# oxfordcontrol/Clarabel.jl

Hardware: AMD Instinct MI355X
Metric: IPM iterations/sec + KKT factor+solve ms, 10k-var sparse QP, 1/2/4/8 GPU (higher is better)
Workload: dtype f64; 1 GPU; random sparse QP n=10000 m=20000 NN cone, uniform pattern (cfg 2a); N=30000, nnzK=99990, nnzL=16225495, supernodes=20125, levels=97, ordering=minimum degree, parallelism=1 independent problem(s), one per GPU

## Files before the change

clarabel.jl_amd/csrc/dense_tile.h:

```cpp
#pragma once
#include <hip/hip_runtime.h>
#include <stdint.h>

#include "device_plan.h"
#include "kernel_util.h"

namespace hipkkt {

template <int NT, int NR>
struct DenseRaw {
    double a[NT], b[NR], d;
};

template <int NT, int NR>
__device__ __forceinline__ void dense_load(DenseRaw<NT, NR> &f, const double *sp, const double *dv, const unsigned (&coff)[NT],
                                           const unsigned (&roff)[NR], unsigned r8, int K, int k0, int lk) {
    int kk = k0 + lk;
    kk = kk < K ? kk : K - 1;
    const unsigned ko = (unsigned)kk * r8;
#ifdef HIPKKT_EXPERIMENT_NOLOAD
    f.d = 1.0 + ko * 1e-9;
#pragma unroll
    for (int t = 0; t < NT; t++) f.a[t] = 1e-3 * (coff[t] + 1);
#pragma unroll
    for (int t = 0; t < NR; t++) f.b[t] = 1e-3 * (roff[t] + 1);
#else
    f.d = ld_off(dv, (unsigned)kk * 8u);
#pragma unroll
    for (int t = 0; t < NT; t++) f.a[t] = ld_off(sp, coff[t] + ko);
#pragma unroll
    for (int t = 0; t < NR; t++) f.b[t] = ld_off(sp, roff[t] + ko);
#endif
}

template <int NT, int NR>
__device__ __forceinline__ void dense_mma(const DenseRaw<NT, NR> &f, v4f64 (&acc)[NT][NR], unsigned mbits, int K, int k0, int lk) {
    const double dk = (k0 + lk < K) ? -f.d : 0.0;
    double a[NT], b[NR];
#pragma unroll
    for (int t = 0; t < NT; t++)
        a[t] = ((mbits >> t) & 1u) ? f.a[t] * dk : 0.0;
#pragma unroll
    for (int t = 0; t < NR; t++) b[t] = ((mbits >> (4 + t)) & 1u) ? f.b[t] : 0.0;
#pragma unroll
    for (int tj = 0; tj < NT; tj++)
#pragma unroll
        for (int ti = 0; ti < NR; ti++)
            acc[tj][ti] = __builtin_amdgcn_mfma_f64_16x16x4f64(a[tj], b[ti], acc[tj][ti], 0, 0, 0);
}

template <int NT, int NR, bool DEEP = false>
__device__ __forceinline__ void dense_tile_core(const DevPlan &P, double *tp, int rt, int nrt, int wt, int task_begin,
                                                int task_end, int lane, int tj0, int ti0) {
    const int l15 = lane & 15, lk = lane >> 4;

    v4f64 acc[NT][NR];
#pragma unroll
    for (int tj = 0; tj < NT; tj++)
#pragma unroll
        for (int reg = 0; reg < 4; reg++) {
            const int jj = (tj0 + tj) * 16 + lk + 4 * reg;
#pragma unroll
            for (int ti = 0; ti < NR; ti++) {
                const int ii = (ti0 + ti) * 16 + l15;
                const bool ok = ii < nrt && jj < wt;
                const double v = ld_off(tp, ok ? (unsigned)(ii + jj * rt) * 8u : 0u);
                acc[tj][ti][reg] = ok ? v : 0.0;
            }
        }

    const int last = task_end - 1;
    auto gm_of = [&](int q, int &g_, int &m_) { const DenseTask *t = P.dtasks + (q < last ? q : last); g_ = t->geom; m_ = t->map; };
    auto req_maps = [&](int geom_u, int map_u, int (&mr_)[NR], int (&mc_)[NT]) {
        const int16_t *tm = P.upd_tmap + (int64_t)((geom_u & (1 << 17)) ? map_u : 0) * 128;
#pragma unroll
        for (int x = 0; x < NR; x++) mr_[x] = tm[(ti0 + x) * 16 + l15];
#pragma unroll
        for (int x = 0; x < NT; x++) mc_[x] = tm[64 + (tj0 + x) * 16 + l15];
    };
    DenseTask Tc = P.dtasks[task_begin];
    int mr[NR], mc[NT], g1, m1;
    req_maps(rfl(Tc.geom), rfl(Tc.map), mr, mc);
    gm_of(task_begin + 1, g1, m1);
    for (int q = task_begin; q < task_end; q++) {
        const DenseTask Tn = P.dtasks[q + 1 < task_end ? q + 1 : q];
        int g2, m2, mrn[NR], mcn[NT];
        gm_of(q + 2, g2, m2);
        req_maps(rfl(g1), rfl(m1), mrn, mcn);
        const int row_lo = rfl(Tc.row_lo), nrows = rfl(Tc.nrows), col_lo = rfl(Tc.col_lo), ncols = rfl(Tc.ncols),
                  geom = rfl(Tc.geom), K = rfl(Tc.K);
        const unsigned r8 = (unsigned)rfl(Tc.r8);
        const double *sp = rfl_ptr(P.Lx + Tc.panel_off);
        const double *dv = rfl_ptr(P.D + Tc.dfirst);
        const int c_r = geom & 255, c_c = (geom >> 8) & 255;
        unsigned roff[NR], coff[NT], mbits = 0;
        if (geom & (1 << 17)) {
#pragma unroll
            for (int x = 0; x < NR; x++) {
                const int m = mr[x];
                roff[x] = (unsigned)(row_lo + (m >= 0 ? m : 0)) * 8u;
                mbits |= m >= 0 ? 16u << x : 0u;
            }
#pragma unroll
            for (int x = 0; x < NT; x++) {
                const int m = mc[x];
                coff[x] = (unsigned)(col_lo + (m >= 0 ? m : 0)) * 8u;
                mbits |= m >= 0 ? 1u << x : 0u;
            }
        } else {
#pragma unroll
            for (int x = 0; x < NR; x++) {
                const int ii = (ti0 + x) * 16 + l15 - c_r;
                const bool okr = ii >= 0 && ii < nrows;
                roff[x] = (unsigned)(row_lo + (okr ? ii : 0)) * 8u;
                mbits |= okr ? 16u << x : 0u;
            }
#pragma unroll
            for (int x = 0; x < NT; x++) {
                const int jj = (tj0 + x) * 16 + l15 - c_c;
                const bool okc = jj >= 0 && jj < ncols;
                coff[x] = (unsigned)(col_lo + (okc ? jj : 0)) * 8u;
                mbits |= okc ? 1u << x : 0u;
            }
        }
        if (NT == 1 || DEEP) {
            DenseRaw<NT, NR> f0, f1, f2, f3;
            dense_load<NT, NR>(f0, sp, dv, coff, roff, r8, K, 0, lk);
            dense_load<NT, NR>(f1, sp, dv, coff, roff, r8, K, 4, lk);
            dense_load<NT, NR>(f2, sp, dv, coff, roff, r8, K, 8, lk);
            dense_load<NT, NR>(f3, sp, dv, coff, roff, r8, K, 12, lk);
            for (int k0 = 0; k0 < K; k0 += 16) {
                __builtin_amdgcn_sched_barrier(0);
                dense_mma<NT, NR>(f0, acc, mbits, K, k0, lk);
                dense_load<NT, NR>(f0, sp, dv, coff, roff, r8, K, k0 + 16, lk);
                __builtin_amdgcn_sched_barrier(0);
                dense_mma<NT, NR>(f1, acc, mbits, K, k0 + 4, lk);
                dense_load<NT, NR>(f1, sp, dv, coff, roff, r8, K, k0 + 20, lk);
                __builtin_amdgcn_sched_barrier(0);
                dense_mma<NT, NR>(f2, acc, mbits, K, k0 + 8, lk);
                dense_load<NT, NR>(f2, sp, dv, coff, roff, r8, K, k0 + 24, lk);
                __builtin_amdgcn_sched_barrier(0);
                dense_mma<NT, NR>(f3, acc, mbits, K, k0 + 12, lk);
                dense_load<NT, NR>(f3, sp, dv, coff, roff, r8, K, k0 + 28, lk);
            }
        } else {
            DenseRaw<NT, NR> fa, fb;
            dense_load<NT, NR>(fa, sp, dv, coff, roff, r8, K, 0, lk);
            for (int k0 = 0; k0 < K; k0 += 8) {
                dense_load<NT, NR>(fb, sp, dv, coff, roff, r8, K, k0 + 4, lk);
                __builtin_amdgcn_sched_barrier(0);
                dense_mma<NT, NR>(fa, acc, mbits, K, k0, lk);
                __builtin_amdgcn_sched_barrier(0);
                dense_load<NT, NR>(fa, sp, dv, coff, roff, r8, K, k0 + 8, lk);
                __builtin_amdgcn_sched_barrier(0);
                if (k0 + 4 < K) dense_mma<NT, NR>(fb, acc, mbits, K, k0 + 4, lk);
                __builtin_amdgcn_sched_barrier(0);
            }
        }
        Tc = Tn;
        g1 = g2; m1 = m2;
#pragma unroll
        for (int x = 0; x < NR; x++) mr[x] = mrn[x];
#pragma unroll
        for (int x = 0; x < NT; x++) mc[x] = mcn[x];
    }
#pragma unroll
    for (int tj = 0; tj < NT; tj++)
#pragma unroll
        for (int reg = 0; reg < 4; reg++) {
            const int jj = (tj0 + tj) * 16 + lk + 4 * reg;
#pragma unroll
            for (int ti = 0; ti < NR; ti++) {
                const int ii = (ti0 + ti) * 16 + l15;
                if (ii < nrt && jj < wt) st_off(tp, (unsigned)(ii + jj * rt) * 8u, acc[tj][ti][reg]);
            }
        }
}

__device__ __forceinline__ void dense_tile_core_full(const DevPlan &P, double *tp, int rt, int task_begin, int task_end, int lane) {
    const int l15 = lane & 15, lk = lane >> 4;
    v4f64 acc[4][4];
#pragma unroll
    for (int tj = 0; tj < 4; tj++)
#pragma unroll
        for (int reg = 0; reg < 4; reg++) {
            const int jj = tj * 16 + lk + 4 * reg;
#pragma unroll
// ... 56 lines not shown
                advance();
            } else if (q + 1 < task_end) {
                const DenseTask Tc = Tn;
                Tn = P.dtasks[q + 2 < task_end ? q + 2 : q + 1];
                setup(Tc);
                load(fa);
                advance();
            }
            __builtin_amdgcn_sched_barrier(0);
            mma(fb);
            __builtin_amdgcn_sched_barrier(0);
        }
    }
#pragma unroll
    for (int tj = 0; tj < 4; tj++)
#pragma unroll
        for (int reg = 0; reg < 4; reg++) {
            const int jj = tj * 16 + lk + 4 * reg;
#pragma unroll
            for (int ti = 0; ti < 4; ti++) st_off(tp, (unsigned)(ti * 16 + l15 + jj * rt) * 8u, acc[tj][ti][reg]);
        }
}

template <int NT, int NR, bool DEEP = false>
__device__ __forceinline__ void dense_tile(const DevPlan &P, const DenseGroup *Gp, int lane, int tj0, int ti0) {
    const DenseGroup G = *Gp;
    const int task_begin = rfl(G.task_begin), task_end = rfl(G.task_end);
    const int wt = rfl(G.wt);
    if (tj0 * 16 >= wt) return;
    const int rt = rfl(G.rt);
    double *tp = rfl_ptr(P.Lx + G.tile_off);
    const int nrt = rfl(G.nrt);
    if (ti0 * 16 >= nrt) return;
    if (NT == 4 && NR == 4 && (rfl(G.pad) & 1)) {
        dense_tile_core_full(P, tp, rt, task_begin, task_end, lane);
        return;
    }
    dense_tile_core<NT, NR, DEEP>(P, tp, rt, nrt, wt, task_begin, task_end, lane, tj0, ti0);
}

__device__ __forceinline__ void dense_extra_tiles(const DevPlan &P, int begin, int count, int xb, int per_wave) {
    const int lane = threadIdx.x & 63;
    int idx = rfl((xb * 4 + (int)(threadIdx.x >> 6)) * per_wave);
    for (int q = 0; q < per_wave && idx < count; q++, idx++) dense_tile<4, 4, true>(P, P.dgroups + begin + idx, lane, 0, 0);
}

}
```

clarabel.jl_amd/csrc/hipkkt_abi.cpp:

```cpp
#include "hipkkt_internal.h"

using namespace hipkkt;
using namespace hipkkt_host;

namespace hipkkt_host {
thread_local std::string g_create_error;
DebugOpts &debug_opts() { static DebugOpts o; return o; }
bool verbose() { static const bool v = getenv("HIPKKT_VERBOSE") != nullptr; return v; }
}

extern "C" {

void hipkkt_default_opts(hipkkt_opts *o) {
    if (!o) return;
    memset(o, 0, sizeof(*o));
    o->index_base = 0;
    o->supernode_max_width = kMaxSnWidth;
    o->relax_supernodes = 1;
    o->update_policy = 2;
    o->update_batch = 0;
    o->front_min_panels = 0;
    o->dynamic_reg_eps = 1e-13;
    o->dynamic_reg_delta = 2e-7;
    o->amd_dense_scale = 1.5;
// ... 670 lines not shown
    else if (k == "FB_V2") o.fb_v2 = !is0();
    else if (k == "FORCE_TWIN") o.force_twin = is1();
    else if (k == "NO_GRAPH") o.no_graph = is1();
    else if (k == "NO_PERSIST") o.no_persist = is1();
    else if (k == "FULL_TILES") o.full_tiles = !is0();
    else if (k == "FRONT_BLOCK") o.front_block = !is0();
    else if (k == "SPLIT_K") o.split_k = !is0();
    else if (k == "GATHER_OVERLAP") o.gather_overlap = !is0();
    else if (k == "GATHER_SORT") o.gather_sort = !is0();
    else if (k == "GATHER_SIDE_BLOCKS") { if (!value) o.gather_side_blocks = def.gather_side_blocks; else if (num(&v) && v >= 0) o.gather_side_blocks = (int)v; else return HIPKKT_ERR_ARGUMENT; }
    else if (k == "DENSE_TRI") o.dense_tri = !is0();
    else if (k == "ORDERING") o.ordering_amd = value && value[0] == 'a';
    else if (k == "NO_FRONT") o.no_front = is1();
    else if (k == "HOST_ASSEMBLY") o.host_assembly = is1();
    else if (k == "FRONT_BLOCK_MIN_ROWS") { if (!value) o.front_block_min_rows = def.front_block_min_rows; else if (num(&v)) o.front_block_min_rows = (int)v; else return HIPKKT_ERR_ARGUMENT; }
    else if (k == "SUPERHOP") { if (!value) o.superhop = def.superhop; else if (num(&v)) o.superhop = (int)v; else return HIPKKT_ERR_ARGUMENT; }
    else if (k == "DEBUG_FLAGS") { if (!value) o.debug_flags = 0; else if (num(&v)) o.debug_flags = (int)v; else return HIPKKT_ERR_ARGUMENT; }
    else if (k == "SPIN_LIMIT") { if (!value) o.spin_limit = def.spin_limit; else if (num(&v) && v >= 0) o.spin_limit = (long long)v; else return HIPKKT_ERR_ARGUMENT; }
    else if (k == "PERSIST_RETRY") { if (!value) o.persist_retry = def.persist_retry; else if (num(&v) && v >= 0) o.persist_retry = (long long)v; else return HIPKKT_ERR_ARGUMENT; }
    else if (k == "ACCURATE") {
        if (!value) o.accurate = def.accurate;
        else if (!num(&v)) return HIPKKT_ERR_ARGUMENT;
        else o.accurate = v == 0.0 ? 1e300 : v;
    } else if (k == "PSD_LARGE_MIN") {
        if (!value) o.psd_large_min = def.psd_large_min;
        else if (!num(&v) || v < 0 || v > 128 || v != (double)(int)v) return HIPKKT_ERR_ARGUMENT;
        else o.psd_large_min = v == 0.0 ? def.psd_large_min : (int)v;
    } else if (k == "FB_EXTRA_PW") {
        o.fb_extra_pw = def.fb_extra_pw; o.fb_pen1 = def.fb_pen1; o.fb_pen2 = def.fb_pen2;
        if (value) {
            int m = o.fb_extra_pw; double a = o.fb_pen1, b = o.fb_pen2;
            if (sscanf(value, "%d,%lf,%lf", &m, &a, &b) < 1) return HIPKKT_ERR_ARGUMENT;
            o.fb_extra_pw = std::max(1, std::min(m, 2)); o.fb_pen1 = a; o.fb_pen2 = b;
        }
    } else {
        g_create_error = "hipkkt_debug_set: unknown switch " + k;
        return HIPKKT_ERR_ARGUMENT;
    }
    return HIPKKT_OK;
#endif
}

const char *hipkkt_last_error(hipkkt_handle h) { return h ? h->err.c_str() : g_create_error.c_str(); }

}
```

clarabel.jl_amd/csrc/hipkkt_factor.cpp:

```cpp
#include "hipkkt_internal.h"

using namespace hipkkt;
using namespace hipkkt_host;

namespace hipkkt_host {

static double slot_value(const hipkkt_solver *S, int slot) {
    double v;
    memcpy(&v, (const char *)S->h_scal + slot * sizeof(double), sizeof(double));
    return v;
}

static void read_scalars(hipkkt_solver *S) {
    HK_CHECK(hipMemcpyAsync(S->h_flags, S->dp.flags, FL_COUNT * sizeof(int), hipMemcpyDeviceToHost, S->stream));
    HK_CHECK(hipMemcpyAsync(S->h_scal, S->dp.scal, SC_COUNT * sizeof(double), hipMemcpyDeviceToHost, S->stream));
    HK_CHECK(hipStreamSynchronize(S->stream));
}


static void enqueue_factor_level(hipkkt_solver *S, int l) {
    const HostPlan &P = S->plan;
    const int n = P.fac_lvl_ptr[l + 1] - P.fac_lvl_ptr[l];
    if (P.fac_lvl_maxw[l] <= 8)
        launch_factor_level(S->stream, S->dp, P.fac_lvl_ptr[l], n, P.fac_lvl_maxw[l], S->opts.dynamic_reg_eps,
                            S->opts.dynamic_reg_delta);
    else
        launch_factor_panel(S->stream, S->dp, P.fac_lvl_ptr[l], n, S->opts.dynamic_reg_eps, S->opts.dynamic_reg_delta);
}

static void enqueue_front_batch(hipkkt_solver *S, const FrontBatch &B) {
#ifdef HIPKKT_TESTING
    if (!S->fb.sw.v2) {
        launch_front_block(S->stream, S->dp, B, S->fb.d_sync, S->fb.d_scratch, S->fb.d_stream, S->opts.dynamic_reg_eps,
                           S->opts.dynamic_reg_delta, S->fb.sw.streamed, S->fb.d_trace);
        return;
    }
#endif
    launch_front_block2(S->stream, S->dp, B, S->fb.d_sync, S->fb.d_scratch, S->fb.d_stream, S->opts.dynamic_reg_eps,
                        S->opts.dynamic_reg_delta, S->fb.d_trace);
}

static void enqueue_split_k(hipkkt_solver *S, int l) {
    if (S->split.group_count[l] <= 0) return;
    launch_update_dense(S->stream, S->dp, S->split.group_begin[l], S->split.group_count[l], false);
    launch_split_reduce(S->stream, S->dp, S->split.d_recs + S->split.rec_ptr[l], S->split.rec_ptr[l + 1] - S->split.rec_ptr[l]);
}

static void enqueue_gather(hipkkt_solver *S, int l) {
    const HostPlan &P = S->plan;
    const int64_t e0 = P.gath_stage_ptr[l], n = P.gath_stage_ptr[l + 1] - e0, h0 = S->split.heavy_ptr[l], nh = S->split.heavy_ptr[l + 1] - h0;
    const int64_t head = S->split.gath[l];
    if (head < 0 || S->side_join_level >= 0) { launch_update_gather(S->stream, S->dp, e0, n, h0, nh); return; }
    const int64_t hh = S->split.gath_heavy[l];
    launch_update_gather(S->stream, S->dp, e0, head, h0, hh);
    HK_CHECK(hipEventRecord(S->ev_fork, S->stream));
    HK_CHECK(hipStreamWaitEvent(S->idle_stream, S->ev_fork, 0));
    launch_update_gather(S->idle_stream, S->dp, e0 + head, n - head, h0 + hh, nh - hh, debug_opts().gather_side_blocks);
    HK_CHECK(hipEventRecord(S->ev_join, S->idle_stream));
    S->side_join_level = l + P.update_batch_used;
}
static void join_side(hipkkt_solver *S, int l) {
    if (S->side_join_level < 0 || l < S->side_join_level) return;
    HK_CHECK(hipStreamWaitEvent(S->stream, S->ev_join, 0));
    S->side_join_level = -1;
}

struct Riders { int count = 0, begin = 0, per_wave = 1; };
// ... 52 lines not shown
        T.prof_dense4_ms = 0; T.prof_dense4_flops = 0; T.prof_dense4_launches = (int)dense.size();
        T.prof_launch_ms.clear(); T.prof_launch_flops.clear(); T.prof_launch_tiles.clear();
        for (const DenseLaunch &d : dense) {
            const double t = ms(d.t);
            T.prof_dense4_ms += t;
            T.prof_dense4_flops += d.flops;
            T.prof_launch_ms.push_back(t);
            T.prof_launch_flops.push_back(d.flops);
            T.prof_launch_tiles.push_back(d.tiles);
        }
        T.prof_fb_ms = 0; T.prof_fb_launches = (int)batches.size(); T.prof_fb_panels = fb_panels; T.prof_fb_flops = fb_flops;
        for (const Span &s : batches) T.prof_fb_ms += ms(s);
        T.prof_extra_tiles = extra_tiles; T.prof_extra_flops = extra_flops;
    }
};

static void enqueue_updates(hipkkt_solver *S, int l, const Riders &x, FactorProbe *probe) {
    const HostPlan &P = S->plan;
    hipStream_t st = S->stream;
    const int g0 = P.upd_stage_ptr[l], nd = P.upd_stage_ndense[l], ng = P.upd_stage_ngather[l];
    if (P.upd_stage_ptr[l + 1] == g0) probe = nullptr;
    if (probe) probe->stage_begin(x);
    join_side(S, l);
    launch_update_dense(st, S->dp, g0, nd - x.count, dense_full_k(nd, P.upd_stage_flops_dense[l]));
    enqueue_split_k(S, l);
    if (probe) probe->dense_end(l, nd - x.count);
    enqueue_gather(S, l);
    launch_update_stage(st, S->dp, g0 + nd + ng, P.upd_stage_ptr[l + 1] - g0 - nd - ng);
    if (probe) probe->stage_end();
}

static double dense_stage_cost_us(int m) {
    if (m <= 0) return 0.0;
    if (m <= kDenseStripTiles) return 20.0 + 0.065 * m;
    if (m <= 768) return 66.0;
    const int k = m / 1024, rem = m % 1024;
    const double base = k == 0 ? 0.0 : k == 1 ? 77.0 : 65.0 * k;
    if (rem == 0) return base;
    if (rem <= 256) return base + 13.0;
    if (rem <= 512) return base + 20.0;
    return k == 0 ? 77.0 : 65.0 * (k + 1);
}
static int fb_extra_tiles_of_stage(int nd, int ncrit, int next_blk, int *per_wave_out) {
    constexpr int cus = 254, rmin = 64;
    const DebugOpts &dbo = debug_opts();
    const int pw_max = dbo.fb_extra_pw;
    const double pen[3] = {0.0, dbo.fb_pen1, dbo.fb_pen2};
// ... 193 lines not shown
```

clarabel.jl_amd/csrc/hipkkt_internal.h:

```cpp
#pragma once
#include "../../include/hipkkt.h"

#include <hip/hip_runtime.h>

#include <algorithm>
#include <atomic>
#include <chrono>
#include <cmath>
#include <cstdlib>
#include <cstring>
#include <deque>
#include <functional>
#include <future>
#include <memory>
#include <mutex>
#include <new>
#include <string>
#include <thread>
#include <vector>

#include "assemble.h"
#include "cone_layout.h"
#include "device_plan.h"
#include "hipkkt_cones.h"
// ... 35 lines not shown
    bool fb_stream = true;
    bool fb_v2 = true;
    bool force_twin = false;
    bool no_graph = false;
    bool no_persist = false;
    bool full_tiles = true;
    bool front_block = true;
    bool split_k = true;
    bool gather_overlap = true;
    bool gather_sort = true;
    int gather_side_blocks = 512;
    bool dense_tri = true;
    bool ordering_amd = false;
    bool no_front = false;
    bool host_assembly = false;
    int front_block_min_rows = -1;
    int superhop = -1;
    int debug_flags = 0;
    long long spin_limit = -1;
    long long persist_retry = -1;
    double accurate = 64.0;
    int fb_extra_pw = 1;
    double fb_pen1 = 10.0, fb_pen2 = 28.0;
    int psd_large_min = 65;
};
DebugOpts &debug_opts();
bool verbose();

struct GraphSlot {
    hipGraphExec_t exec = nullptr;
    bool valid = false;
    int static_enable = -1;
    double eps_const = 0, eps_prop = 0;
};

}

using namespace hipkkt;
using namespace hipkkt_host;

struct RefineOpts {
    int32_t enable; double reltol, abstol; int64_t max_iter; double stop_ratio;
    bool same_graph(const RefineOpts &o) const { return reltol == o.reltol && abstol == o.abstol && max_iter == o.max_iter && stop_ratio == o.stop_ratio; }
};

constexpr int kNumCtx = 2;
// ... 24 lines not shown
    bool l1 = false;
    KKTImage img;
    HostPlan plan;
    PlanOptions plan_opts;
    SolveSchedule sched;
    DevPlan dp{};
    std::vector<std::pair<void *, size_t>> allocs;
    std::string err;

    int N = 0;
    int64_t nnzK = 0;
    std::chrono::steady_clock::time_point t_created{};
    PersistState persist;
    FrontBatchState fb;
    UpdateSplit split;
    SocTables soc;
    ResidualBuffers res;
    ReducedSolve red;
    TwinState twin;
    SolverStats stats;
    ConeState cones;
    double accurate_threshold = 64.0;
    int last_npolish = 0;
    int inv_nsmall = 0, inv_wsmall = 1, inv_nwide = 0;
    int side_join_level = -1;
    hipEvent_t ev_fork = nullptr, ev_join = nullptr;

    int64_t *d_mapHs = nullptr, *d_mapP = nullptr, *d_mapA = nullptr, *d_diag_full = nullptr;
    std::vector<int64_t> cone_numel;
    std::vector<int32_t> cone_hs_dense, cone_sparse_kind;

    double *d_stage = nullptr;
    int64_t *d_stage_idx = nullptr;
    int64_t stage_cap = 0;
    double *h_scal = nullptr;
    double *h_scal_red = nullptr;
    int *h_flags = nullptr;

    hipkkt_host::GraphSlot g_factor;
    bool use_graph = true;
    bool runtime_ready = false;
    bool profiling = false;
    bool profiling_no_extra = false;
    hipEvent_t ev0 = nullptr, ev1 = nullptr, ev2 = nullptr, ev3 = nullptr;
    bool kval_event_pending = false;
    double last_eps = 0;
// ... 129 lines not shown
```

clarabel.jl_amd/csrc/hipkkt_setup.cpp:

```cpp
#include "hipkkt_internal.h"

using namespace hipkkt;
using namespace hipkkt_host;

namespace hipkkt_host {

namespace {
struct PlanCache {
    struct Entry {
        uint64_t key;
        std::string optkey;
        std::vector<int64_t> colptr, rowval;
        std::shared_ptr<const HostPlan> plan;
    };
    std::mutex mu;
    std::deque<Entry> entries;
    int64_t hits = 0, misses = 0;
    static constexpr size_t kMaxEntries = 8;
    static constexpr int64_t kMaxNnzL = 40000000;
    static PlanCache &get() { static PlanCache c; return c; }
    static bool enabled() { return debug_opts().plan_cache; }
    static uint64_t fnv(uint64_t h, const void *p, size_t n) {
        const unsigned char *b = (const unsigned char *)p;
        for (size_t i = 0; i < n; i++) { h ^= b[i]; h *= 1099511628211ull; }
// ... 16 lines not shown
};
}
void plan_cache_counts(int64_t *hits, int64_t *misses) {
    PlanCache &c = PlanCache::get();
    std::lock_guard<std::mutex> lk(c.mu);
    *hits = c.hits; *misses = c.misses;
}

void init_runtime(hipkkt_solver *S) {
    HK_CHECK(hipSetDevice(S->device));
    RuntimePool &rp = RuntimePool::get();
    auto need = [&](void *p) { if (!p) throw DeviceError{"creating a stream / event / pinned buffer failed"}; return p; };
    S->stream = (hipStream_t)need(rp.stream_get(S->device, 0));
    S->idle_stream = (hipStream_t)need(rp.stream_get(S->device, 1));
    {
        const DebugOpts &o = debug_opts();
        S->fb.sw.extra = o.fb_extra;
        S->fb.sw.streamed = o.fb_stream;
        S->fb.sw.v2 = o.fb_v2 && S->fb.sw.streamed;
#ifndef HIPKKT_TESTING
        S->fb.sw.streamed = S->fb.sw.v2 = true;
#endif
        S->accurate_threshold = o.accurate;
        S->twin.force = o.force_twin;
    }
    static_assert(SC_COUNT * sizeof(double) <= RuntimePool::kPinned && sizeof(RefineState) <= RuntimePool::kPinned, "pinned chunk too small");
    for (hipEvent_t *e : {&S->ev0, &S->ev1, &S->ev2, &S->ev3, &S->ev_fork, &S->ev_join}) *e = (hipEvent_t)need(rp.event_get(S->device));
    S->h_scal = (double *)need(rp.pinned_alloc(S->device));
    S->h_flags = (int *)need(rp.pinned_alloc(S->device));
    S->h_scal_red = S->h_scal + 16;
    static_assert((16 + kScalRedDoubles) * sizeof(double) <= RuntimePool::kPinned, "pinned chunk too small for the reduced-solve scalars");
    memset(S->h_scal, 0, SC_COUNT * sizeof(double));
    memset(S->h_flags, 0, FL_COUNT * sizeof(int));
    if (debug_opts().no_graph) S->use_graph = false;
    for (int c = 0; c < kNumCtx; c++) {
        SolveCtx &C = S->ctx[c];
        if (c == 0) C.stream = S->stream;
        else { C.stream = (hipStream_t)need(rp.stream_get(S->device, 2)); C.own_stream = true; }
        C.ev_a = (hipEvent_t)need(rp.event_get(S->device));
        C.ev_b = (hipEvent_t)need(rp.event_get(S->device));
        C.h_rs = (RefineState *)need(rp.pinned_alloc(S->device));
        C.h_flags = (int *)need(rp.pinned_alloc(S->device));
        memset(C.h_rs, 0, sizeof(RefineState));
        memset(C.h_flags, 0, FL_COUNT * sizeof(int));
    }
}
// ... 536 lines not shown
```

clarabel.jl_amd/csrc/kernel_util.h:

```cpp
#pragma once
#include <hip/hip_runtime.h>
#include <stdint.h>

namespace hipkkt {

static inline unsigned nblk(int64_t n, int bs = 256) { return (unsigned)((n + bs - 1) / bs); }

typedef double v4f64 __attribute__((ext_vector_type(4)));

__device__ __forceinline__ double readlane_f64(double x, int l) {
    const unsigned long long u = (unsigned long long)__double_as_longlong(x);
    const unsigned lo = __builtin_amdgcn_readlane((unsigned)u, l), hi = __builtin_amdgcn_readlane((unsigned)(u >> 32), l);
    return __longlong_as_double((long long)(((unsigned long long)hi << 32) | lo));
}
__device__ __forceinline__ int rfl(int v) { return __builtin_amdgcn_readfirstlane(v); }

template <class T>
__device__ __forceinline__ T *rfl_ptr(T *p) {
    const unsigned long long u = (unsigned long long)p;
    const unsigned lo = __builtin_amdgcn_readfirstlane((unsigned)u), hi = __builtin_amdgcn_readfirstlane((unsigned)(u >> 32));
    return (T *)(((unsigned long long)hi << 32) | lo);
}
#define HK_GLOBAL __attribute__((address_space(1)))
__device__ __forceinline__ double ld_off(const double *base, unsigned byte_off) {
    return *(const HK_GLOBAL double *)((const HK_GLOBAL char *)base + byte_off);
}
__device__ __forceinline__ void st_off(double *base, unsigned byte_off, double v) {
    *(HK_GLOBAL double *)((HK_GLOBAL char *)base + byte_off) = v;
}

__device__ __forceinline__ int ld_relaxed_i(const int *p) { return __hip_atomic_load(p, __ATOMIC_RELAXED, __HIP_MEMORY_SCOPE_AGENT); }
__device__ __forceinline__ double ld_relaxed(const double *p) { return __hip_atomic_load(p, __ATOMIC_RELAXED, __HIP_MEMORY_SCOPE_AGENT); }
__device__ __forceinline__ void st_relaxed(double *p, double v) { __hip_atomic_store(p, v, __ATOMIC_RELAXED, __HIP_MEMORY_SCOPE_AGENT); }

__device__ __forceinline__ double pivot_rcp(double d) {
    double r = __builtin_amdgcn_rcp(d);
    r = fma(fma(-d, r, 1.0), r, r);
    r = fma(fma(-d, r, 1.0), r, r);
    return r;
}

__device__ __forceinline__ double pivot_rcp3(double d) {
    const double r = __builtin_amdgcn_rcp(d);
    const double e = fma(-d, r, 1.0);
    const double e2 = fma(e, e, e);
    return fma(r, e2, r);
// ... 38 lines not shown
```

clarabel.jl_amd/csrc/kernels.h:

```cpp
#pragma once
#include <hip/hip_runtime.h>

#include "device_plan.h"

namespace hipkkt {
void launch_scatter_values(hipStream_t st, double *kval, const int64_t *idx, const double *vals, int64_t n, double scale);
void launch_scale_values(hipStream_t st, double *kval, const int64_t *idx, int64_t n, double scale);
void launch_soc_batch(hipStream_t st, double *kval, const int64_t *uidx, const int64_t *vidx, const int *cone_of,
                      const double *u, const double *v, const double *eta2, int64_t n, const int64_t *didx, int nsoc);
void launch_psd_hs(hipStream_t st, double *kval, const int64_t *map_hs, int64_t hs_off, const double *W, int n, const int *skip = nullptr);
void launch_zero_words(hipStream_t st, void *p, int nwords);
void launch_maxabs_gather(hipStream_t st, const double *v, const int64_t *idx, int64_t n, unsigned long long *slot);
void launch_init_panels(hipStream_t st, const DevPlan &P, int64_t nnz, int static_enable, double eps_const, double eps_prop);
void launch_factor_level(hipStream_t st, const DevPlan &P, int item_begin, int nitems, int wmax, double dyn_eps, double dyn_delta);
void launch_factor_panel(hipStream_t st, const DevPlan &P, int item_begin, int nitems, double dyn_eps, double dyn_delta);
void launch_update_stage(hipStream_t st, const DevPlan &P, int group_begin, int ngroups);
constexpr int kDenseStripTiles = 384;
constexpr double kFullKFlopsPerTile = 1.5e6;
inline bool dense_full_k(int nd, double flops) { return nd > 0 && flops >= kFullKFlopsPerTile * nd; }
void launch_update_dense(hipStream_t st, const DevPlan &P, int group_begin, int ngroups, bool full_k = false);
void launch_split_reduce(hipStream_t st, const DevPlan &P, const SplitRec *recs, int n);
void launch_update_gather(hipStream_t st, const DevPlan &P, int64_t ebegin, int64_t n, int64_t hbegin, int64_t nheavy, int max_blocks = 0);
void launch_invert_diag(hipStream_t st, const DevPlan &P, int n_small, int wmax_small, int n_wide);
void launch_permute_in(hipStream_t st, const double *b, const int *perm, double *y, int n, int *epoch, int *ticks, int nticks, int *zero = nullptr,
                       int nzero = 0);
void launch_fwd_level(hipStream_t st, const DevPlan &P, int item_begin, int nitems, double *y, double *z);
void launch_bwd_partial(hipStream_t st, const DevPlan &P, int item_begin, int nitems, const double *x);
void launch_bwd_final(hipStream_t st, const DevPlan &P, int sn_begin, int nsn, const double *z, double *x, double *xout);
void launch_fwd_narrow(hipStream_t st, const DevPlan &P, int sn_begin, int n, int wmax, double *y, double *z);
void launch_bwd_narrow(hipStream_t st, const DevPlan &P, int sn_begin, int n, int wmax, const double *z, double *x, double *xout);
void launch_fwd_seg(hipStream_t st, const DevPlan &P, int seg, int item_begin, int nitems, int nsuper, double *y, double *z);
void launch_bwd_seg(hipStream_t st, const DevPlan &P, int seg, int item_begin, int nitems, int nsuper, int first, const double *z,
                    double *x, double *xout);
void launch_front_fwd(hipStream_t st, const DevPlan &P, const FrontDesc &F, double *y, double *z);
void launch_front_bwd(hipStream_t st, const DevPlan &P, const FrontDesc &F, const double *z, double *x, double *xout);
void launch_invert_super(hipStream_t st, const DevPlan &P, const FrontDesc &F);
void launch_spmv_residual(hipStream_t st, const DevPlan &P, const double *b, const RefineState *rs, const double *x0, const double *x1,
                          double *e, int n, unsigned long long *slot);
int long_row_threshold();
void launch_norm_inf(hipStream_t st, const double *v, int n, unsigned long long *slot);
void launch_refine_decide(hipStream_t st, RefineState *rs, const double *scal, int phase, double reltol, double abstol, int max_iter,
                          double stop_ratio);
void launch_refine_add(hipStream_t st, const RefineState *rs, double *x0, double *x1, const double *corr, int n);
// ... 118 lines not shown
```

clarabel.jl_amd/csrc/kernels.hip:

```cpp
#include <hip/hip_runtime.h>
#include <stdint.h>
#include <type_traits>

#include "device_plan.h"
#include "kernel_util.h"
#include "kernels.h"
#include "dense_tile.h"

namespace hipkkt {

__global__ void k_maxabs_gather(const double *__restrict__ v, const int64_t *__restrict__ idx, int64_t n,
                                unsigned long long *__restrict__ slot) {
    int64_t i = (int64_t)blockIdx.x * blockDim.x + threadIdx.x;
    double a = 0.0;
    if (i < n) a = fabs(idx ? v[idx[i]] : v[i]);
    block_atomic_max_abs(slot, a);
}

__global__ void k_init_panels(double *__restrict__ Lx, const double *__restrict__ kval,
                              const int64_t *__restrict__ kmap, const signed char *__restrict__ kdiag_sign,
                              int64_t nnz, const double *__restrict__ scal, int static_enable,
                              double eps_const, double eps_prop) {
    int64_t q = (int64_t)blockIdx.x * blockDim.x + threadIdx.x;
    if (q >= nnz) return;
// ... 456 lines not shown
            for (int reg = 0; reg < 4; reg++) {
                const int ii = tmi * 16 + lk + 4 * reg;
                rp[tmi * 4 + reg] = (ii < T.nrows && cp >= 0) ? rel[(T.row_lo + ii) - T.col_lo] - G.row_base : -1;
            }
        while (__atomic_load_n(&turn, __ATOMIC_RELAXED) != v) __builtin_amdgcn_s_sleep(1);
        __builtin_amdgcn_fence(__ATOMIC_ACQUIRE, "workgroup");
#pragma unroll
        for (int tmi = 0; tmi < 4; tmi++)
#pragma unroll
            for (int reg = 0; reg < 4; reg++) {
                const int rr = rp[tmi * 4 + reg];
                if (rr >= 0) Ct[cp * LDC + rr] -= acc[tmi][reg];
            }
        __builtin_amdgcn_fence(__ATOMIC_RELEASE, "workgroup");
        if (lane == 0) __atomic_store_n(&turn, v + 1, __ATOMIC_RELAXED);
    }
    __syncthreads();
    for (int idx = tid; idx < nrt * wt; idx += kUpdWaves * 64) {
        int row = idx % nrt, col = idx / nrt;
        tp[(G.row_base + row) + (int64_t)col * rt] = Ct[col * LDC + row];
    }
}

template <int NT, int NR>
__global__ void __launch_bounds__(256, NT == 2 ? 4 : 2)
k_update_dense(DevPlan P, int group_begin, int ngroups) {
    static_assert(NR == 4 || NT == 1, "rows are split only between the workgroups of a one-strip-per-wave launch");
    const int lane = threadIdx.x & 63;
    const int wave = rfl(threadIdx.x >> 6);
    const int tj0 = (wave % (4 / NT)) * NT;
    if (NR == 4) {
        for (int g = rfl(blockIdx.x * NT + wave / (4 / NT)); g < ngroups; g += gridDim.x * NT)
            dense_tile<NT, NR>(P, P.dgroups + group_begin + g, lane, tj0, 0);
    } else {
        constexpr int RS = 4 / NR;
        for (int u = blockIdx.x; u < ngroups * RS; u += gridDim.x)
            dense_tile<NT, NR>(P, P.dgroups + group_begin + u / RS, lane, tj0, (u % RS) * NR);
    }
}

template <int PIECES>
__global__ void __launch_bounds__(256, 2)
k_update_dense_tail(DevPlan P, int group_begin, int nfull, int ngroups) {
    const int lane = threadIdx.x & 63;
    const int wave = rfl(threadIdx.x >> 6);
    const int nfw = nfull >> 2;
    if ((int)blockIdx.x < nfw) {
        dense_tile<4, 4>(P, P.dgroups + group_begin + rfl(blockIdx.x * 4 + wave), lane, 0, 0);
    } else if (PIECES == 4) {
        const int g = nfull + ((int)blockIdx.x - nfw);
        if (g < ngroups) dense_tile<1, 4>(P, P.dgroups + group_begin + g, lane, wave, 0);
    } else {
        const int g = nfull + 2 * ((int)blockIdx.x - nfw) + (wave >> 1);
        if (g < ngroups) dense_tile<2, 4>(P, P.dgroups + group_begin + g, lane, (wave & 1) * 2, 0);
    }
}

__device__ __forceinline__ double gath_pair_sum(const DevPlan &P, const GathPair &G, double acc) {
    const double *li = P.Lx + G.src;
    const double *lj = li + G.dj;
// ... 48 lines not shown
    if (lane == 0) P.Lx[P.gath_tgt[e]] -= acc;
}

void launch_maxabs_gather(hipStream_t st, const double *v, const int64_t *idx, int64_t n, unsigned long long *slot) {
    if (n > 0) hipLaunchKernelGGL(k_maxabs_gather, dim3(nblk(n)), dim3(256), 0, st, v, idx, n, slot);
}
void launch_init_panels(hipStream_t st, const DevPlan &P, int64_t nnz, int static_enable, double eps_const, double eps_prop) {
    if (nnz > 0)
        hipLaunchKernelGGL(k_init_panels, dim3(nblk(nnz)), dim3(256), 0, st, P.Lx, P.kval, P.kmap, P.kdiag_sign, nnz,
                           P.scal, static_enable, eps_const, eps_prop);
}
static size_t factor_lds_bytes(int wmax) { return sizeof(double) * (size_t)(wmax * (wmax + 1) + wmax + wmax * LDT); }
void launch_factor_level(hipStream_t st, const DevPlan &P, int item_begin, int nitems, int wmax, double dyn_eps, double dyn_delta) {
    if (nitems > 0)
        hipLaunchKernelGGL(k_factor_level, dim3(nitems), dim3(256), factor_lds_bytes(wmax), st, P, item_begin, wmax, dyn_eps,
                           dyn_delta);
}
void launch_factor_panel(hipStream_t st, const DevPlan &P, int item_begin, int nitems, double dyn_eps, double dyn_delta) {
    if (nitems > 0) hipLaunchKernelGGL(k_factor_panel, dim3(nitems), dim3(512), 0, st, P, item_begin, dyn_eps, dyn_delta);
}
void launch_update_stage(hipStream_t st, const DevPlan &P, int group_begin, int ngroups) {
    if (ngroups > 0) hipLaunchKernelGGL(k_update_stage, dim3(ngroups), dim3(kUpdWaves * 64), 0, st, P, group_begin);
}
void launch_update_dense(hipStream_t st, const DevPlan &P, int group_begin, int ngroups, bool full_k) {
    if (ngroups <= 0) return;
    if (ngroups > kDenseStripTiles) {
        const int round = 1024, r = ngroups % round, nfull = ngroups - r;
        if (full_k && r > 0 && (r <= 256 || (nfull == 0 && r <= 768)))
            hipLaunchKernelGGL(k_update_dense_tail<4>, dim3(nfull / 4 + r), dim3(256), 0, st, P, group_begin, nfull, ngroups);
        else if (full_k && r > 0 && r <= 512)
            hipLaunchKernelGGL(k_update_dense_tail<2>, dim3(nfull / 4 + (r + 1) / 2), dim3(256), 0, st, P, group_begin, nfull, ngroups);
        else
            hipLaunchKernelGGL((k_update_dense<4, 4>), dim3((ngroups + 3) / 4), dim3(256), 0, st, P, group_begin, ngroups);
    } else {
        hipLaunchKernelGGL((k_update_dense<1, 2>), dim3(ngroups * 2), dim3(256), 0, st, P, group_begin, ngroups);
    }
}
__global__ void __launch_bounds__(256)
k_split_reduce(DevPlan P, const SplitRec *recs) {
    const SplitRec R = recs[blockIdx.x];
    double *tp = P.Lx + R.tile_off, *sc = P.Lx + R.scratch_off;
    for (int idx = threadIdx.x; idx < 4096; idx += 256) {
        const int row = idx & 63, col = idx >> 6;
        double s = 0.0;
        for (int q = 0; q < R.nparts; q++) {
            s += sc[(int64_t)q * 4096 + idx];
            sc[(int64_t)q * 4096 + idx] = 0.0;
        }
        if (row < R.nrt && col < R.wt) tp[row + (int64_t)col * R.rt] += s;
    }
}
void launch_split_reduce(hipStream_t st, const DevPlan &P, const SplitRec *recs, int n) {
    if (n > 0) hipLaunchKernelGGL(k_split_reduce, dim3(n), dim3(256), 0, st, P, recs);
}
void launch_update_gather(hipStream_t st, const DevPlan &P, int64_t ebegin, int64_t n, int64_t hbegin, int64_t nheavy, int max_blocks) {
    if (n > 0) hipLaunchKernelGGL(k_update_gather, dim3(max_blocks > 0 ? std::min<unsigned>(nblk(n), (unsigned)max_blocks) : nblk(n)), dim3(256), 0, st, P, ebegin, n);
    if (nheavy > 0) hipLaunchKernelGGL(k_update_gather_heavy, dim3(nblk(nheavy, 4)), dim3(256), 0, st, P, hbegin, nheavy);
}
// ... 9 lines not shown
```

clarabel.jl_amd/hipkkt.py:

```python
from __future__ import annotations

import ctypes as C
import os

import numpy as np

_HERE = os.path.dirname(os.path.abspath(__file__))
_TESTING = os.environ.get("CLARABEL_HIPKKT_TESTING", "0") == "1"
LIB_PATH = os.environ.get("CLARABEL_HIPKKT_LIB", os.path.join(_HERE, "libclarabel_hipkkt_testing.so" if _TESTING else "libclarabel_hipkkt.so"))

DEBUG_KEYS = ["PLAN_CACHE", "FB_EXTRA", "FB_STREAM", "FB_V2", "FORCE_TWIN", "NO_GRAPH", "NO_PERSIST", "FULL_TILES", "FRONT_BLOCK", "SPLIT_K",
              "DENSE_TRI", "ORDERING", "NO_FRONT", "HOST_ASSEMBLY", "FRONT_BLOCK_MIN_ROWS", "SUPERHOP", "DEBUG_FLAGS", "SPIN_LIMIT",
              "PERSIST_RETRY", "ACCURATE", "FB_EXTRA_PW", "GATHER_OVERLAP", "GATHER_SIDE_BLOCKS", "GATHER_SORT", "PSD_LARGE_MIN"]

_i64p = np.ctypeslib.ndpointer(dtype=np.int64, flags="C_CONTIGUOUS")
_i32p = np.ctypeslib.ndpointer(dtype=np.int32, flags="C_CONTIGUOUS")
_f64p = np.ctypeslib.ndpointer(dtype=np.float64, flags="C_CONTIGUOUS")

ABI_VERSION = 5

SYMBOLS = [
    "hipkkt_default_opts", "hipkkt_is_available", "hipkkt_abi_version", "hipkkt_trim_cache", "hipkkt_create", "hipkkt_create_from_parts", "hipkkt_destroy",
    "hipkkt_get_dims", "hipkkt_info", "hipkkt_get_cost_model", "hipkkt_get_kkt", "hipkkt_get_perm",
    "hipkkt_get_dsigns", "hipkkt_get_map", "hipkkt_get_sparse_map", "hipkkt_update_values", "hipkkt_scale_values",
    "hipkkt_set_hs", "hipkkt_set_hs_dev", "hipkkt_set_hs_psd", "hipkkt_set_cone_types", "hipkkt_update_scaling", "hipkkt_update_scaling_dev", "hipkkt_set_cone_types_ex", "hipkkt_get_nonsym_len", "hipkkt_update_scaling_ex", "hipkkt_update_scaling_ex_dev", "hipkkt_block_products", "hipkkt_set_soc", "hipkkt_set_soc_batch", "hipkkt_set_genpow",
    "hipkkt_update_P", "hipkkt_update_A", "hipkkt_refactor", "hipkkt_setrhs", "hipkkt_setrhs_dev", "hipkkt_solve",
    "hipkkt_solve_dev", "hipkkt_solve_multi", "hipkkt_solve_multi_dev", "hipkkt_kkt_solve_reduced", "hipkkt_kkt_solve_reduced_dev", "hipkkt_ldl_solve", "hipkkt_get_timing", "hipkkt_reset_timing", "hipkkt_get_profile", "hipkkt_get_profile_launches", "hipkkt_set_profiling",
    "hipkkt_get_counters", "hipkkt_debug_dump", "hipkkt_debug_extra_tiles", "hipkkt_debug_set", "hipkkt_debug_is_testing_build", "hipkkt_set_qb", "hipkkt_residuals", "hipkkt_residuals_dev",
    "hipkkt_selftest_mfma", "hipkkt_box_probe", "hipkkt_last_error",
    "hipkkt_cone_affine_ds", "hipkkt_cone_combined_ds_shift", "hipkkt_cone_ds_from_dz_offset", "hipkkt_cone_mul_hs", "hipkkt_cone_step_length",
    "hipkkt_set_equilibration", "hipkkt_step_affine_dev", "hipkkt_step_combined_dev", "hipkkt_step_apply_dev", "hipkkt_step_info_norms_dev",
    "hipkkt_step_get",
    "hipkkt_step_enable_cone3", "hipkkt_cone_barrier", "hipkkt_step_barrier_dev", "hipkkt_step_enable_genpow",
    "hipkkt_step_enable_psd", "hipkkt_psd_set_factors", "hipkkt_psd_set_factors_dev",
    "hipkkt_psd_scaling_enable", "hipkkt_psd_get_factors",
    "hipkkt_cone_set_identity_scaling", "hipkkt_cone_margins", "hipkkt_cone_shift_to_interior", "hipkkt_step_default_start_dev",
# ... 794 lines not shown
```

Measured before the change: 212.7 IPM-iterations/s (KKT iteration units: 1 update + 1 factor + 3 refined solves [constant-rhs + affine concurrently, then combined], inputs in HBM).

## Stream 1x2 dense strip update through a 16-deep cross-task load ring

The small-group dense update kernel (k_update_dense<1,2>) now runs a continuous software pipeline. A ring of 16 in-flight K-slices keeps loads going across task boundaries instead of draining and refilling a 4-deep pipeline for each task. Task records are read with scalar constant-address loads, and map lookups are skipped for unmapped tasks. The aim is to hide HBM latency on short-K tasks, at the cost of more registers held by the ring and possible occupancy loss. The old 4-deep form stays available behind a STRIP_RING=4 debug option.

Result: no change. 210.9 IPM-iterations/s (KKT iteration units: 1 update + 1 factor + 3 refined solves [constant-rhs + affine concurrently, then combined], inputs in HBM) (-0.9%).

```diff
diff --git a/clarabel.jl_amd/csrc/dense_tile.h b/clarabel.jl_amd/csrc/dense_tile.h
--- a/clarabel.jl_amd/csrc/dense_tile.h
+++ b/clarabel.jl_amd/csrc/dense_tile.h
@@ -34,8 +34,7 @@
 }
 
 template <int NT, int NR>
-__device__ __forceinline__ void dense_mma(const DenseRaw<NT, NR> &f, v4f64 (&acc)[NT][NR], unsigned mbits, int K, int k0, int lk) {
-    const double dk = (k0 + lk < K) ? -f.d : 0.0;
+__device__ __forceinline__ void dense_mma(const DenseRaw<NT, NR> &f, v4f64 (&acc)[NT][NR], unsigned mbits, double dk) {
     double a[NT], b[NR];
 #pragma unroll
     for (int t = 0; t < NT; t++)
@@ -48,8 +47,14 @@
         for (int ti = 0; ti < NR; ti++)
             acc[tj][ti] = __builtin_amdgcn_mfma_f64_16x16x4f64(a[tj], b[ti], acc[tj][ti], 0, 0, 0);
 }
-
-template <int NT, int NR, bool DEEP = false>
+template <int NT, int NR>
+__device__ __forceinline__ void dense_mma(const DenseRaw<NT, NR> &f, v4f64 (&acc)[NT][NR], unsigned mbits, int K, int k0, int lk) {
+    dense_mma<NT, NR>(f, acc, mbits, (k0 + lk < K) ? -f.d : 0.0);
+}
+
+constexpr int kStripRing12 = 16;
+
+template <int NT, int NR, bool DEEP = false, int RING = 4, bool STREAM = false>
 __device__ __forceinline__ void dense_tile_core(const DevPlan &P, double *tp, int rt, int nrt, int wt, int task_begin,
                                                 int task_end, int lane, int tj0, int ti0) {
     const int l15 = lane & 15, lk = lane >> 4;
@@ -70,40 +75,49 @@
         }
 
     const int last = task_end - 1;
-    auto gm_of = [&](int q, int &g_, int &m_) { const DenseTask *t = P.dtasks + (q < last ? q : last); g_ = t->geom; m_ = t->map; };
-    auto req_maps = [&](int geom_u, int map_u, int (&mr_)[NR], int (&mc_)[NT]) {
-        const int16_t *tm = P.upd_tmap + (int64_t)((geom_u & (1 << 17)) ? map_u : 0) * 128;
-#pragma unroll
-        for (int x = 0; x < NR; x++) mr_[x] = tm[(ti0 + x) * 16 + l15];
-#pragma unroll
-        for (int x = 0; x < NT; x++) mc_[x] = tm[64 + (tj0 + x) * 16 + l15];
-    };
-    DenseTask Tc = P.dtasks[task_begin];
-    int mr[NR], mc[NT], g1, m1;
+    auto rec_of = [&](int i) { return STREAM ? ld_uniform(P.dtasks + i) : P.dtasks[i]; };
+    auto gm_of = [&](int q, int &g_, int &m_) {
+        const DenseTask *t = P.dtasks + (q < last ? q : last);
+        g_ = STREAM ? ld_uniform(&t->geom) : t->geom;
+        m_ = STREAM ? ld_uniform(&t->map) : t->map;
+    };
+    auto req_maps = [&](int geom_u, int map_u, unsigned (&mr_)[NR], unsigned (&mc_)[NT]) {
+        const bool mapped = geom_u & (1 << 17);
+        const uint16_t *tm = (const uint16_t *)P.upd_tmap + (int64_t)(mapped ? map_u : 0) * 128;
+        if (!STREAM || mapped) {
+#pragma unroll
+            for (int x = 0; x < NR; x++) mr_[x] = tm[(ti0 + x) * 16 + l15];
+#pragma unroll
+            for (int x = 0; x < NT; x++) mc_[x] = tm[64 + (tj0 + x) * 16 + l15];
+        }
+    };
+    DenseTask Tc = rec_of(task_begin);
+    unsigned mr[NR], mc[NT];
+    int g1, m1;
     req_maps(rfl(Tc.geom), rfl(Tc.map), mr, mc);
     gm_of(task_begin + 1, g1, m1);
-    for (int q = task_begin; q < task_end; q++) {
-        const DenseTask Tn = P.dtasks[q + 1 < task_end ? q + 1 : q];
-        int g2, m2, mrn[NR], mcn[NT];
-        gm_of(q + 2, g2, m2);
-        req_maps(rfl(g1), rfl(m1), mrn, mcn);
+    unsigned roff[NR], coff[NT], mbits, r8;
+    const double *sp, *dv;
+    int K, q = task_begin;
+    auto begin_task = [&]() {
         const int row_lo = rfl(Tc.row_lo), nrows = rfl(Tc.nrows), col_lo = rfl(Tc.col_lo), ncols = rfl(Tc.ncols),
-                  geom = rfl(Tc.geom), K = rfl(Tc.K);
-        const unsigned r8 = (unsigned)rfl(Tc.r8);
-        const double *sp = rfl_ptr(P.Lx + Tc.panel_off);
-        const double *dv = rfl_ptr(P.D + Tc.dfirst);
+                  geom = rfl(Tc.geom);
+        K = rfl(Tc.K);
+        r8 = (unsigned)rfl(Tc.r8);
+        sp = rfl_ptr(P.Lx + Tc.panel_off);
+        dv = rfl_ptr(P.D + Tc.dfirst);
         const int c_r = geom & 255, c_c = (geom >> 8) & 255;
-        unsigned roff[NR], coff[NT], mbits = 0;
+        mbits = 0;
         if (geom & (1 << 17)) {
 #pragma unroll
             for (int x = 0; x < NR; x++) {
-                const int m = mr[x];
+                const int m = (int16_t)mr[x];
                 roff[x] = (unsigned)(row_lo + (m >= 0 ? m : 0)) * 8u;
                 mbits |= m >= 0 ? 16u << x : 0u;
             }
 #pragma unroll
             for (int x = 0; x < NT; x++) {
-                const int m = mc[x];
+                const int m = (int16_t)mc[x];
                 coff[x] = (unsigned)(col_lo + (m >= 0 ? m : 0)) * 8u;
                 mbits |= m >= 0 ? 1u << x : 0u;
             }
@@ -123,27 +137,68 @@
                 mbits |= okc ? 1u << x : 0u;
             }
         }
-        if (NT == 1 || DEEP) {
-            DenseRaw<NT, NR> f0, f1, f2, f3;
-            dense_load<NT, NR>(f0, sp, dv, coff, roff, r8, K, 0, lk);
-            dense_load<NT, NR>(f1, sp, dv, coff, roff, r8, K, 4, lk);
-            dense_load<NT, NR>(f2, sp, dv, coff, roff, r8, K, 8, lk);
-            dense_load<NT, NR>(f3, sp, dv, coff, roff, r8, K, 12, lk);
-            for (int k0 = 0; k0 < K; k0 += 16) {
-                __builtin_amdgcn_sched_barrier(0);
-                dense_mma<NT, NR>(f0, acc, mbits, K, k0, lk);
-                dense_load<NT, NR>(f0, sp, dv, coff, roff, r8, K, k0 + 16, lk);
-                __builtin_amdgcn_sched_barrier(0);
-                dense_mma<NT, NR>(f1, acc, mbits, K, k0 + 4, lk);
-                dense_load<NT, NR>(f1, sp, dv, coff, roff, r8, K, k0 + 20, lk);
-                __builtin_amdgcn_sched_barrier(0);
-                dense_mma<NT, NR>(f2, acc, mbits, K, k0 + 8, lk);
-                dense_load<NT, NR>(f2, sp, dv, coff, roff, r8, K, k0 + 24, lk);
-                __builtin_amdgcn_sched_barrier(0);
-                dense_mma<NT, NR>(f3, acc, mbits, K, k0 + 12, lk);
-                dense_load<NT, NR>(f3, sp, dv, coff, roff, r8, K, k0 + 28, lk);
+        const int gn = rfl(g1), mn = rfl(m1);
+        Tc = rec_of(q + 1 < task_end ? q + 1 : q);
+        gm_of(q + 2, g1, m1);
+        req_maps(gn, mn, mr, mc);
+        q++;
+    };
+    if (NT == 1 || DEEP) {
+        DenseRaw<NT, NR> f[RING];
+        if (STREAM) {
+            unsigned fm[RING];
+            int kp;
+            int nv;
+            auto issue = [&](DenseRaw<NT, NR> &fs, unsigned &ms) {
+                dense_load<NT, NR>(fs, sp, dv, coff, roff, r8, K, kp, lk);
+                ms = kp + lk < K ? mbits : 0u;
+                nv += kp < K ? 1 : 0;
+                kp += 4;
+                if (kp >= K && q < task_end) {
+                    begin_task();
+                    kp = 0;
+                }
+            };
+            auto all_requested = [&]() { return kp >= K && q >= task_end; };
+            if (q < task_end) {
+                begin_task();
+                kp = 0;
+                nv = 0;
+#pragma unroll
+                for (int s = 0; s < RING; s++) issue(f[s], fm[s]);
+                while (!all_requested()) {
+                    nv = 0;
+#pragma unroll
+                    for (int s = 0; s < RING; s++) {
+                        __builtin_amdgcn_sched_barrier(0);
+                        dense_mma<NT, NR>(f[s], acc, fm[s], -f[s].d);
+                        issue(f[s], fm[s]);
+                    }
+                }
+#pragma unroll
+                for (int s = 0; s < RING; s++) {
+                    __builtin_amdgcn_sched_barrier(0);
+                    if (s < nv) dense_mma<NT, NR>(f[s], acc, fm[s], -f[s].d);
+                }
             }
         } else {
+            while (q < task_end) {
+                begin_task();
+#pragma unroll
+                for (int s = 0; s < RING; s++) dense_load<NT, NR>(f[s], sp, dv, coff, roff, r8, K, 4 * s, lk);
+                for (int k0 = 0; k0 < K; k0 += 4 * RING) {
+#pragma unroll
+                    for (int s = 0; s < RING; s++) {
+                        __builtin_amdgcn_sched_barrier(0);
+                        dense_mma<NT, NR>(f[s], acc, mbits, K, k0 + 4 * s, lk);
+                        dense_load<NT, NR>(f[s], sp, dv, coff, roff, r8, K, k0 + 4 * (RING + s), lk);
+                    }
+                }
+            }
+        }
+    } else {
+        while (q < task_end) {
+            begin_task();
             DenseRaw<NT, NR> fa, fb;
             dense_load<NT, NR>(fa, sp, dv, coff, roff, r8, K, 0, lk);
             for (int k0 = 0; k0 < K; k0 += 8) {
@@ -157,12 +212,6 @@
                 __builtin_amdgcn_sched_barrier(0);
             }
         }
-        Tc = Tn;
-        g1 = g2; m1 = m2;
-#pragma unroll
-        for (int x = 0; x < NR; x++) mr[x] = mrn[x];
-#pragma unroll
-        for (int x = 0; x < NT; x++) mc[x] = mcn[x];
     }
 #pragma unroll
     for (int tj = 0; tj < NT; tj++)
@@ -265,7 +314,7 @@
         }
 }
 
-template <int NT, int NR, bool DEEP = false>
+template <int NT, int NR, bool DEEP = false, int RING = 4, bool STREAM = false>
 __device__ __forceinline__ void dense_tile(const DevPlan &P, const DenseGroup *Gp, int lane, int tj0, int ti0) {
     const DenseGroup G = *Gp;
     const int task_begin = rfl(G.task_begin), task_end = rfl(G.task_end);
@@ -279,7 +328,7 @@
         dense_tile_core_full(P, tp, rt, task_begin, task_end, lane);
         return;
     }
-    dense_tile_core<NT, NR, DEEP>(P, tp, rt, nrt, wt, task_begin, task_end, lane, tj0, ti0);
+    dense_tile_core<NT, NR, DEEP, RING, STREAM>(P, tp, rt, nrt, wt, task_begin, task_end, lane, tj0, ti0);
 }
 
 __device__ __forceinline__ void dense_extra_tiles(const DevPlan &P, int begin, int count, int xb, int per_wave) {
diff --git a/clarabel.jl_amd/csrc/hipkkt_abi.cpp b/clarabel.jl_amd/csrc/hipkkt_abi.cpp
--- a/clarabel.jl_amd/csrc/hipkkt_abi.cpp
+++ b/clarabel.jl_amd/csrc/hipkkt_abi.cpp
@@ -716,6 +716,10 @@
         if (!value) o.accurate = def.accurate;
         else if (!num(&v)) return HIPKKT_ERR_ARGUMENT;
         else o.accurate = v == 0.0 ? 1e300 : v;
+    } else if (k == "STRIP_RING") {
+        if (!value) o.strip_ring = def.strip_ring;
+        else if (!num(&v) || (v != 0.0 && v != 4.0)) return HIPKKT_ERR_ARGUMENT;
+        else o.strip_ring = (int)v;
     } else if (k == "PSD_LARGE_MIN") {
         if (!value) o.psd_large_min = def.psd_large_min;
         else if (!num(&v) || v < 0 || v > 128 || v != (double)(int)v) return HIPKKT_ERR_ARGUMENT;
diff --git a/clarabel.jl_amd/csrc/hipkkt_factor.cpp b/clarabel.jl_amd/csrc/hipkkt_factor.cpp
--- a/clarabel.jl_amd/csrc/hipkkt_factor.cpp
+++ b/clarabel.jl_amd/csrc/hipkkt_factor.cpp
@@ -42,7 +42,7 @@
 
 static void enqueue_split_k(hipkkt_solver *S, int l) {
     if (S->split.group_count[l] <= 0) return;
-    launch_update_dense(S->stream, S->dp, S->split.group_begin[l], S->split.group_count[l], false);
+    launch_update_dense(S->stream, S->dp, S->split.group_begin[l], S->split.group_count[l], false, S->strip_ring);
     launch_split_reduce(S->stream, S->dp, S->split.d_recs + S->split.rec_ptr[l], S->split.rec_ptr[l + 1] - S->split.rec_ptr[l]);
 }
 
@@ -141,7 +141,7 @@
     if (P.upd_stage_ptr[l + 1] == g0) probe = nullptr;
     if (probe) probe->stage_begin(x);
     join_side(S, l);
-    launch_update_dense(st, S->dp, g0, nd - x.count, dense_full_k(nd, P.upd_stage_flops_dense[l]));
+    launch_update_dense(st, S->dp, g0, nd - x.count, dense_full_k(nd, P.upd_stage_flops_dense[l]), S->strip_ring);
     enqueue_split_k(S, l);
     if (probe) probe->dense_end(l, nd - x.count);
     enqueue_gather(S, l);
diff --git a/clarabel.jl_amd/csrc/hipkkt_internal.h b/clarabel.jl_amd/csrc/hipkkt_internal.h
--- a/clarabel.jl_amd/csrc/hipkkt_internal.h
+++ b/clarabel.jl_amd/csrc/hipkkt_internal.h
@@ -81,6 +81,7 @@
     double accurate = 64.0;
     int fb_extra_pw = 1;
     double fb_pen1 = 10.0, fb_pen2 = 28.0;
+    int strip_ring = 0;
     int psd_large_min = 65;
 };
 DebugOpts &debug_opts();
@@ -151,6 +152,7 @@
     ConeState cones;
     double accurate_threshold = 64.0;
     int last_npolish = 0;
+    int strip_ring = 0;
     int inv_nsmall = 0, inv_wsmall = 1, inv_nwide = 0;
     int side_join_level = -1;
     hipEvent_t ev_fork = nullptr, ev_join = nullptr;
diff --git a/clarabel.jl_amd/csrc/hipkkt_setup.cpp b/clarabel.jl_amd/csrc/hipkkt_setup.cpp
--- a/clarabel.jl_amd/csrc/hipkkt_setup.cpp
+++ b/clarabel.jl_amd/csrc/hipkkt_setup.cpp
@@ -62,6 +62,7 @@
         S->fb.sw.streamed = S->fb.sw.v2 = true;
 #endif
         S->accurate_threshold = o.accurate;
+        S->strip_ring = o.strip_ring;
         S->twin.force = o.force_twin;
     }
     static_assert(SC_COUNT * sizeof(double) <= RuntimePool::kPinned && sizeof(RefineState) <= RuntimePool::kPinned, "pinned chunk too small");
diff --git a/clarabel.jl_amd/csrc/kernel_util.h b/clarabel.jl_amd/csrc/kernel_util.h
--- a/clarabel.jl_amd/csrc/kernel_util.h
+++ b/clarabel.jl_amd/csrc/kernel_util.h
@@ -22,6 +22,16 @@
     return (T *)(((unsigned long long)hi << 32) | lo);
 }
 #define HK_GLOBAL __attribute__((address_space(1)))
+#define HK_CONSTANT __attribute__((address_space(4)))
+template <class T>
+__device__ __forceinline__ T ld_uniform(const T *p) {
+    static_assert(sizeof(T) % 4 == 0 && alignof(T) >= 4, "whole words");
+    const HK_CONSTANT unsigned *w = (const HK_CONSTANT unsigned *)(unsigned long long)rfl_ptr(p);
+    union { T v; unsigned u[sizeof(T) / 4]; } r;
+#pragma unroll
+    for (unsigned i = 0; i < sizeof(T) / 4; i++) r.u[i] = w[i];
+    return r.v;
+}
 __device__ __forceinline__ double ld_off(const double *base, unsigned byte_off) {
     return *(const HK_GLOBAL double *)((const HK_GLOBAL char *)base + byte_off);
 }
diff --git a/clarabel.jl_amd/csrc/kernels.h b/clarabel.jl_amd/csrc/kernels.h
--- a/clarabel.jl_amd/csrc/kernels.h
+++ b/clarabel.jl_amd/csrc/kernels.h
@@ -18,7 +18,7 @@
 constexpr int kDenseStripTiles = 384;
 constexpr double kFullKFlopsPerTile = 1.5e6;
 inline bool dense_full_k(int nd, double flops) { return nd > 0 && flops >= kFullKFlopsPerTile * nd; }
-void launch_update_dense(hipStream_t st, const DevPlan &P, int group_begin, int ngroups, bool full_k = false);
+void launch_update_dense(hipStream_t st, const DevPlan &P, int group_begin, int ngroups, bool full_k = false, int strip_ring = 0);
 void launch_split_reduce(hipStream_t st, const DevPlan &P, const SplitRec *recs, int n);
 void launch_update_gather(hipStream_t st, const DevPlan &P, int64_t ebegin, int64_t n, int64_t hbegin, int64_t nheavy, int max_blocks = 0);
 void launch_invert_diag(hipStream_t st, const DevPlan &P, int n_small, int wmax_small, int n_wide);
diff --git a/clarabel.jl_amd/csrc/kernels.hip b/clarabel.jl_amd/csrc/kernels.hip
--- a/clarabel.jl_amd/csrc/kernels.hip
+++ b/clarabel.jl_amd/csrc/kernels.hip
@@ -502,7 +502,7 @@
     }
 }
 
-template <int NT, int NR>
+template <int NT, int NR, int RING = 4, bool STREAM = false>
 __global__ void __launch_bounds__(256, NT == 2 ? 4 : 2)
 k_update_dense(DevPlan P, int group_begin, int ngroups) {
     static_assert(NR == 4 || NT == 1, "rows are split only between the workgroups of a one-strip-per-wave launch");
@@ -511,11 +511,11 @@
     const int tj0 = (wave % (4 / NT)) * NT;
     if (NR == 4) {
         for (int g = rfl(blockIdx.x * NT + wave / (4 / NT)); g < ngroups; g += gridDim.x * NT)
-            dense_tile<NT, NR>(P, P.dgroups + group_begin + g, lane, tj0, 0);
+            dense_tile<NT, NR, false, RING, STREAM>(P, P.dgroups + group_begin + g, lane, tj0, 0);
     } else {
         constexpr int RS = 4 / NR;
         for (int u = blockIdx.x; u < ngroups * RS; u += gridDim.x)
-            dense_tile<NT, NR>(P, P.dgroups + group_begin + u / RS, lane, tj0, (u % RS) * NR);
+            dense_tile<NT, NR, false, RING, STREAM>(P, P.dgroups + group_begin + u / RS, lane, tj0, (u % RS) * NR);
     }
 }
 
@@ -610,8 +610,9 @@
 void launch_update_stage(hipStream_t st, const DevPlan &P, int group_begin, int ngroups) {
     if (ngroups > 0) hipLaunchKernelGGL(k_update_stage, dim3(ngroups), dim3(kUpdWaves * 64), 0, st, P, group_begin);
 }
-void launch_update_dense(hipStream_t st, const DevPlan &P, int group_begin, int ngroups, bool full_k) {
+void launch_update_dense(hipStream_t st, const DevPlan &P, int group_begin, int ngroups, bool full_k, int strip_ring) {
     if (ngroups <= 0) return;
+    const bool first_form = strip_ring == 4;
     if (ngroups > kDenseStripTiles) {
         const int round = 1024, r = ngroups % round, nfull = ngroups - r;
         if (full_k && r > 0 && (r <= 256 || (nfull == 0 && r <= 768)))
@@ -620,8 +621,10 @@
             hipLaunchKernelGGL(k_update_dense_tail<2>, dim3(nfull / 4 + (r + 1) / 2), dim3(256), 0, st, P, group_begin, nfull, ngroups);
         else
             hipLaunchKernelGGL((k_update_dense<4, 4>), dim3((ngroups + 3) / 4), dim3(256), 0, st, P, group_begin, ngroups);
+    } else if (first_form) {
+        hipLaunchKernelGGL((k_update_dense<1, 2>), dim3(ngroups * 2), dim3(256), 0, st, P, group_begin, ngroups);
     } else {
-        hipLaunchKernelGGL((k_update_dense<1, 2>), dim3(ngroups * 2), dim3(256), 0, st, P, group_begin, ngroups);
+        hipLaunchKernelGGL((k_update_dense<1, 2, kStripRing12, true>), dim3(ngroups * 2), dim3(256), 0, st, P, group_begin, ngroups);
     }
 }
 __global__ void __launch_bounds__(256)
diff --git a/clarabel.jl_amd/hipkkt.py b/clarabel.jl_amd/hipkkt.py
--- a/clarabel.jl_amd/hipkkt.py
+++ b/clarabel.jl_amd/hipkkt.py
@@ -11,7 +11,7 @@
 
 DEBUG_KEYS = ["PLAN_CACHE", "FB_EXTRA", "FB_STREAM", "FB_V2", "FORCE_TWIN", "NO_GRAPH", "NO_PERSIST", "FULL_TILES", "FRONT_BLOCK", "SPLIT_K",
               "DENSE_TRI", "ORDERING", "NO_FRONT", "HOST_ASSEMBLY", "FRONT_BLOCK_MIN_ROWS", "SUPERHOP", "DEBUG_FLAGS", "SPIN_LIMIT",
-              "PERSIST_RETRY", "ACCURATE", "FB_EXTRA_PW", "GATHER_OVERLAP", "GATHER_SIDE_BLOCKS", "GATHER_SORT", "PSD_LARGE_MIN"]
+              "PERSIST_RETRY", "ACCURATE", "FB_EXTRA_PW", "GATHER_OVERLAP", "GATHER_SIDE_BLOCKS", "GATHER_SORT", "PSD_LARGE_MIN", "STRIP_RING"]
 
 _i64p = np.ctypeslib.ndpointer(dtype=np.int64, flags="C_CONTIGUOUS")
 _i32p = np.ctypeslib.ndpointer(dtype=np.int32, flags="C_CONTIGUOUS")
```
